# emuell/AFEC

Hardware: AMD Instinct MI355X
Metric: audio frames/sec low-level crawl, 44.1kHz 1024-hop (higher is better)
Workload: dtype f64

## Files before the change

### afec_amd/csrc/afx_frames32.hip

```cpp

#include <hip/hip_runtime.h>

#include "afx_internal.h"
#include "afx_device.h"
#include "afx_fft32.h"

namespace afx {
namespace {

using f32x32::cx;

constexpr int kHalfSlots = 1056;
constexpr int kPlane32Bytes = 2 * kHalfSlots * 8;
constexpr int kWaves32 = 8;

template <int POST_ROWS>
struct Lds32 {
  static constexpr int tw = 0;
  static constexpr int post = tw + 32 * 32 * 16;
  static constexpr int dct = post + POST_ROWS * 32 * 16;
  static constexpr int logc = dct + 14 * 16 * 8;
  static constexpr int xchg = logc + 32 * 8;
  static constexpr int total = xchg + kWaves32 * kPlane32Bytes;
};

__device__ __forceinline__ __amdgpu_buffer_rsrc_t table_rsrc(const void* p, int bytes) {
  return __builtin_amdgcn_make_buffer_rsrc(const_cast<void*>(p), 0, bytes, 0x00020000);
}
typedef unsigned int u32x4_t __attribute__((ext_vector_type(4)));
typedef unsigned int u32x2_t __attribute__((ext_vector_type(2)));
__device__ __forceinline__ double2 table_load2(__amdgpu_buffer_rsrc_t rs, int lane_off, int row_off) {
  return __builtin_bit_cast(double2, __builtin_amdgcn_raw_buffer_load_b128(rs, lane_off, row_off, 0));
}
__device__ __forceinline__ double table_load1(__amdgpu_buffer_rsrc_t rs, int lane_off, int row_off) {
  return __builtin_bit_cast(double, __builtin_amdgcn_raw_buffer_load_b64(rs, lane_off, row_off, 0));
}

template <int IMM, bool NT>
__device__ __forceinline__ void dma_piece(const void* gaddr, unsigned lds_base) {
  if constexpr (NT)
    asm volatile("s_mov_b32 m0, %1\n\ts_nop 0\n\tglobal_load_lds_dwordx4 %0, off offset:%2 nt"
                 :: "v"(gaddr), "s"(lds_base), "n"(IMM) : "memory", "m0");
  else
    asm volatile("s_mov_b32 m0, %1\n\ts_nop 0\n\tglobal_load_lds_dwordx4 %0, off offset:%2"
                 :: "v"(gaddr), "s"(lds_base), "n"(IMM) : "memory", "m0");
}
template <bool NT = true>
__device__ __forceinline__ void dma_hop(const float* g, unsigned lds_plane) {
  dma_piece<0, NT>(g, lds_plane);
  dma_piece<512, NT>(g, lds_plane + 512);
  dma_piece<1024, NT>(g, lds_plane + 1024);
  dma_piece<1536, NT>(g, lds_plane + 1536);
  dma_piece<2048, NT>(g, lds_plane + 2048);
  dma_piece<2560, NT>(g, lds_plane + 2560);
  dma_piece<3072, NT>(g, lds_plane + 3072);
  dma_piece<3584, NT>(g, lds_plane + 3584);
}

__device__ __forceinline__ double mag_sqrt_mel(double xr, double xi, double tiny, double three) {
  const double x = fma(xi, xi, fma(xr, xr, tiny));
  const double r = __builtin_amdgcn_rsq(x);
  const double y = x * r;
  return y * fma(-r, y, three);
}

__device__ __forceinline__ void keep_lane0(double& re, double& im, double own_re, double own_im, unsigned long long lane0_mask) {
  unsigned long long saved;
  asm volatile("s_mov_b64 %2, exec\n\ts_mov_b64 exec, %5\n\tv_mov_b64 %0, %3\n\tv_mov_b64 %1, %4\n\ts_mov_b64 exec, %2"
               : "+v"(re), "+v"(im), "=&s"(saved) : "v"(own_re), "v"(own_im), "s"(lane0_mask));
}

__device__ __forceinline__ double half_sum16(double (&a)[16], int lane) {
#pragma unroll
  for (int i = 0; i < 8; ++i) {
    swap16(a[i], a[i + 8]);
    a[i] += a[i + 8];
  }
  const bool b3 = (lane & 8) != 0, b2 = (lane & 4) != 0, b1 = (lane & 2) != 0;
#pragma unroll
  for (int i = 0; i < 4; ++i) {
    const double keep = b3 ? a[i + 4] : a[i];
    const double send = b3 ? a[i] : a[i + 4];
    a[i] = keep + dpp_mov<kDppRor8>(send);
  }
#pragma unroll
  for (int i = 0; i < 2; ++i) {
    const double keep = b2 ? a[i + 2] : a[i];
    const double send = b2 ? a[i] : a[i + 2];
    a[i] = keep + dpp_mov<kDppHalfMirror>(send);
  }
  const double keep = b1 ? a[1] : a[0];
  const double send = b1 ? a[0] : a[1];
  double z = keep + dpp_mov<kDppXor2>(send);
  z += dpp_mov<kDppXor1>(z);
  return z;
}

__device__ const double kLogConst[32] = {1.0 / 23.0, 1.0 / 21.0, 1.0 / 19.0, 1.0 / 17.0, 1.0 / 15.0, 1.0 / 13.0,
                                         1.0 / 11.0, 1.0 / 9.0,  1.0 / 7.0,  1.0 / 5.0,  1.0 / 3.0,  0.693147180559945309417,
                                         0.70710678118654752440, 2e-42,
                                         1e-20, 32.0, 0.38268343236508984, -0.9238795325112867, 1.0 / 738.0,
                                         (double)(85.0f / 100.0), 43.0, -1.0 / 60.0, (double)1e-12f, 3.0,
                                         1.44269504088896340736, 20.0 / 2.30258509299404568402, 2.2250738585072014e-308, 3.33547137486383e-154 , 511.0, 0.0, 0.0, 0.0};
constexpr int kCEps = 14, kC32 = 15, kCRotRe = 16, kCRotIm = 17, kCRoll = 19, kCSqrtMin = 27, kC511 = 28;

__device__ __forceinline__ double log_lds(double x, const double* c) {
  double m = __builtin_amdgcn_frexp_mant(x);
  int e = __builtin_amdgcn_frexp_exp(x);
  const bool lowhalf = m < c[12];
  m = lowhalf ? m + m : m;
  e = lowhalf ? e - 1 : e;
  const double s = fast_div(m - 1.0, m + 1.0);
  const double z = s * s;
  double p = c[0];
#pragma unroll
  for (int i = 1; i < 11; ++i) p = fma(p, z, c[i]);
  p = fma(p, z, 1.0);
  return fma((double)e, c[11], 2.0 * s * p);
}

__device__ __forceinline__ void finish_mfcc32(double acc, double*& recp, int& left, int stride2, const double* dct,
                                              const double* logc, int lane) {
  const double lg = log_lds(fmax(acc, logc[13]), logc);
  int ln = lane;
  asm volatile("" : "+v"(ln));
  const int n = (ln >> 1) & 15;
  const double2* drow = reinterpret_cast<const double2*>(dct + 16 * (n < kNumCep ? n : 0));
  const int idx = ((ln & 32) + (ln & 1)) << 2;
  const int lo32 = __double2loint(lg), hi32 = __double2hiint(lg);
  double c = 0.0;
#pragma unroll
  for (int m = 0; m < kNumCep; m += 2) {
    const double2 d = drow[m >> 1];
    const double l0 = __hiloint2double(__builtin_amdgcn_ds_bpermute(idx + 8 * m, hi32), __builtin_amdgcn_ds_bpermute(idx + 8 * m, lo32));
    const double l1 = __hiloint2double(__builtin_amdgcn_ds_bpermute(idx + 8 * m + 8, hi32), __builtin_amdgcn_ds_bpermute(idx + 8 * m + 8, lo32));
    c = fma(l0, d.x, c);
    c = fma(l1, d.y, c);
  }
  if (n < kNumCep && left > 0) *recp = c;
  recp += stride2;
  left -= 2;
}

#ifndef AFX_STAMPS
#define AFX_STAMPS 0
#endif
#if AFX_STAMPS
#define AFX_STAMP(i)                                                                           \
  do {                                                                                         \
    unsigned long long t_;                                                                     \
    asm volatile("s_memtime %0\n\ts_waitcnt lgkmcnt(0)" : "=s"(t_));                           \
    stamp_acc[i] += (unsigned)(t_ - stamp_prev);                                               \
    stamp_prev = t_;                                                                           \
  } while (0)
#else
#define AFX_STAMP(i)
#endif


template <int FEAT, bool SCALED>
__global__ __launch_bounds__(kWaves32 * 64) void frames32_kernel(const FrameArgs a) {
  constexpr bool MAGS = (FEAT == 4 || FEAT == 6);
  constexpr bool MAGS_UPPER = (FEAT == 4);
  constexpr int kMelEarly = 4;
  constexpr bool LO_LDS = (FEAT >= 2 && FEAT <= 4) || FEAT == 6;
  constexpr bool kHopNt = !LO_LDS;
  constexpr bool kLoNt = true;
  constexpr bool STATS = (FEAT >= 1 && FEAT <= 3) || FEAT == 5;
  constexpr bool MOMENTS34 = (FEAT != 5);
  constexpr bool PAIRS = STATS;
  constexpr bool STORE = (FEAT == 2 || FEAT == 3);
  constexpr bool UPPER = (FEAT == 3);
  constexpr int MR = (FEAT >= 1) ? 16 : kMel32Rows;
  using Map = Lds32<kMel32Rows>;
  extern __shared__ __align__(16) unsigned char lds_raw[];
  const int lane = threadIdx.x & 63;
  const int wave = __builtin_amdgcn_readfirstlane(threadIdx.x >> 6);
  const int h = lane >> 5, q = lane & 31;

  copy_lds_table(lds_raw + Map::tw, a.tw32, 32 * 32 * 16, threadIdx.x, kWaves32 * 64);
  copy_lds_table(lds_raw + Map::post, a.post32, kMel32Rows * 32 * 16, threadIdx.x, kWaves32 * 64);
  copy_lds_table(lds_raw + Map::dct, a.dct, 14 * 16 * 8, threadIdx.x, kWaves32 * 64);
  copy_lds_table(lds_raw + Map::logc, kLogConst, 32 * 8, threadIdx.x, kWaves32 * 64);
#if AFX_STAMPS
  unsigned stamp_acc[16] = {};
  unsigned long long life_core0, life_real0;
  asm volatile("s_memtime %0\n\ts_memrealtime %1\n\ts_waitcnt lgkmcnt(0)" : "=s"(life_core0), "=s"(life_real0));
  const bool stamping = (wave == 0) && a.stamps != nullptr;
  unsigned long long stamp_prev = 0;
#endif
  __syncthreads();

  const __amdgpu_buffer_rsrc_t win_rs = table_rsrc(a.win32, 32 * 32 * 16);
  const __amdgpu_buffer_rsrc_t mel_rs = table_rsrc(a.melw32, kMel32Pairs * 32 * 8);
  const int q16 = 16 * q, q8 = 8 * q;
  const double2* const tw = reinterpret_cast<const double2*>(lds_raw + Map::tw) + q;
  const double2* const post = reinterpret_cast<const double2*>(lds_raw + Map::post) + q;
  const double* const dct = reinterpret_cast<const double*>(lds_raw + Map::dct);
  const double* const logc = reinterpret_cast<const double*>(lds_raw + Map::logc);
  const int stride2 = 2 * a.lay.stride;
  double* const plane = reinterpret_cast<double*>(lds_raw + Map::xchg + wave * kPlane32Bytes) + kHalfSlots * h;
  double* const pw = plane + q;
  using lds_vdouble = volatile __attribute__((address_space(3))) double;
  lds_vdouble* const pr = (lds_vdouble*)(plane + 33 * q);
  const int partner = (lane & 32) + ((32 - q) & 31);
  const int dh = (lane >> 4) & 1, drow = lane >> 5, dq = 2 * (lane & 15);
  typedef __attribute__((address_space(3))) void lvoid;
  unsigned char* const plane_bytes = lds_raw + Map::xchg + wave * kPlane32Bytes;
  const unsigned plane_lds = __builtin_amdgcn_readfirstlane((unsigned)(size_t)(lvoid*)plane_bytes);
  double k_tiny = 2.2250738585072014e-308, k_three = 3.0;
  unsigned long long k_lane0 = 0x0000000100000001ull;
  asm volatile("" : "+s"(k_tiny), "+s"(k_three), "+s"(k_lane0));
  lds_vdouble* const hop = (lds_vdouble*)(plane_bytes + 256 * h + 8 * q);

  const float* const pcm = reinterpret_cast<const float*>(a.pcm);

  const int n_items = (a.n_chunks + 1) >> 1;
  const int n_static = min((int)(gridDim.x * kWaves32), n_items);
  for (int slot = blockIdx.x * kWaves32 + wave; slot < n_items;) {
    const int ci = 2 * slot + h;
    const bool have = ci < a.n_chunks;
    const Chunk ch = a.chunks[have ? ci : 2 * slot];
    const int nfr = have ? ch.nframes : 0;
    const double sc = ch.scale;
    const int total = max(__builtin_amdgcn_readlane(nfr, 0), __builtin_amdgcn_readlane(nfr, 32));
    const float2* src = reinterpret_cast<const float2*>(pcm + ch.sample_off) + q;
    const int cid = 2 * slot + dh;
    const bool have_d = cid < a.n_chunks;
    const Chunk chd = a.chunks[have_d ? cid : 2 * slot];
    const int last_d = max((have_d ? (int)chd.nframes : 0) - 1, 0);
    const float* const dsrc = pcm + chd.sample_off + 64 * (16 + drow) + 2 * dq;

    double lo[16];
    if constexpr (!LO_LDS) {
      const double* const src8 = reinterpret_cast<const double*>(src);
#pragma unroll
      for (int r = 0; r < 16; ++r) lo[r] = src8[32 * r];
    } else {
      dma_hop<kLoNt>(dsrc - kHop, plane_lds + 8192);
    }
    dma_hop<kHopNt>(dsrc, plane_lds);

    double mel_acc = 0.0;
    double* recp = a.rec + ((int64_t)ch.frame0 + (q & 1)) * a.lay.stride + a.lay.mfcc + ((q >> 1) & 15);
    int left = nfr - (q & 1);

    double2 w[32];
#pragma unroll
    for (int r = 0; r < 32; ++r) w[r] = table_load2(win_rs, q16, 512 * r);

#if AFX_STAMPS
    asm volatile("s_memtime %0\n\ts_waitcnt lgkmcnt(0)" : "=s"(stamp_prev));
#endif
    for (int fi = 0; fi < total; ++fi) {
      cx<double> v[32];
      {
        double nx[16];
        asm volatile("s_waitcnt vmcnt(0)" ::: "memory");
        AFX_STAMP(0);
#pragma unroll
        for (int r = 0; r < 16; ++r) nx[r] = hop[64 * r];
        __builtin_amdgcn_sched_barrier(0);
        if constexpr (LO_LDS) {
          const double* const lo_rows = reinterpret_cast<const double*>(plane_bytes + 8192 + 256 * h) + q;
#pragma unroll
          for (int r = 0; r < 16; ++r) lo[r] = lo_rows[64 * r];
        }
        double hop_sq = 0.0, hop_max = 0.0;
#pragma unroll
        for (int j = 0; j < 8; ++j) {
          auto first = [](double pair) { return __int_as_float(__double2loint(pair)); };
          auto second = [](double pair) { return __int_as_float(__double2hiint(pair)); };
          const double ar = pcm_double<SCALED>(first(lo[j]), sc), ai = pcm_double<SCALED>(second(lo[j]), sc);
          const double br = pcm_double<SCALED>(first(lo[j + 8]), sc), bi = pcm_double<SCALED>(second(lo[j + 8]), sc);
          const double cr = pcm_double<SCALED>(first(nx[j]), sc), ci = pcm_double<SCALED>(second(nx[j]), sc);
          const double dr = pcm_double<SCALED>(first(nx[j + 8]), sc), di = pcm_double<SCALED>(second(nx[j + 8]), sc);
          if constexpr (MAGS) {
            hop_sq = fma(ar, ar, fma(ai, ai, fma(br, br, fma(bi, bi, hop_sq))));
            hop_max = fmax(fmax(hop_max, fmax(fabs(ar), fabs(ai))), fmax(fabs(br), fabs(bi)));
          }
          const double par = ar * w[j].x, pai = ai * w[j].y, pbr = br * w[j + 8].x, pbi = bi * w[j + 8].y;
          const double t0r = fma(cr, w[j + 16].x, par), t0i = fma(ci, w[j + 16].y, pai);
          const double t1r = fma(-cr, w[j + 16].x, par), t1i = fma(-ci, w[j + 16].y, pai);
          const double t2r = fma(dr, w[j + 24].x, pbr), t2i = fma(di, w[j + 24].y, pbi);
          const double t3r = fma(-dr, w[j + 24].x, pbr), t3i = fma(-di, w[j + 24].y, pbi);
          v[j] = {t0r + t2r, t0i + t2i};
          v[j + 16] = {t0r - t2r, t0i - t2i};
          v[j + 8] = {t1r + t3i, t1i - t3r};
          v[j + 24] = {t1r - t3i, t1i + t3r};
        }
        if constexpr (!LO_LDS) {
#pragma unroll
          for (int r = 0; r < 16; ++r) lo[r] = nx[r];
        }
        if constexpr (MAGS) {
          if (a.mask & ((1u << 11) | (1u << 12))) {
            hop_sq += dpp_or_zero<kDppXor1>(hop_sq);      hop_max = fmax(hop_max, dpp_mov<kDppXor1>(hop_max));
            hop_sq += dpp_or_zero<kDppXor2>(hop_sq);      hop_max = fmax(hop_max, dpp_mov<kDppXor2>(hop_max));
            hop_sq += dpp_or_zero<kDppHalfMirror>(hop_sq); hop_max = fmax(hop_max, dpp_mov<kDppHalfMirror>(hop_max));
            hop_sq += dpp_or_zero<kDppMirror>(hop_sq);    hop_max = fmax(hop_max, dpp_mov<kDppMirror>(hop_max));
            const double sq_h = h ? read_lane<32>(hop_sq) + read_lane<48>(hop_sq) : read_lane<0>(hop_sq) + read_lane<16>(hop_sq);
            const double mx_h = h ? fmax(read_lane<32>(hop_max), read_lane<48>(hop_max)) : fmax(read_lane<0>(hop_max), read_lane<16>(hop_max));
            if (q == 0 && fi < nfr) {
              double* const rec = a.rec + ((int64_t)ch.frame0 + fi) * a.lay.stride;
              if ((a.mask & (1u << 11)) && a.lay.amp_peak >= 0) rec[a.lay.amp_peak] = mx_h;
              if ((a.mask & (1u << 12)) && a.lay.amp_rms >= 0) rec[a.lay.amp_rms] = nan_to_zero(sqrt(sq_h / (double)kHop));
            }
          }
        }
      }
      __builtin_amdgcn_sched_barrier(0);
      AFX_STAMP(1);
      f32x32::dft32_rest(v);
      __builtin_amdgcn_sched_barrier(0);
      AFX_STAMP(2);

      double2 t[32];
      auto load_tw = [&](int g) {
#pragma unroll
        for (int j = 2 * g; j < 2 * g + 2; ++j)
#pragma unroll
          for (int i = 0; i < 4; ++i)
            if (j + 8 * i != 0) t[j + 8 * i] = tw[32 * (j + 8 * i)];
      };
      auto bfly_tw = [&](int g) {
#pragma unroll
        for (int j = 2 * g; j < 2 * g + 2; ++j) {
          const cx<double> w1{t[j + 8].x, t[j + 8].y}, w2{t[j + 16].x, t[j + 16].y}, w3{t[j + 24].x, t[j + 24].y};
          if (j == 0) f32x32::radix4_tw3(v[0], v[8], v[16], v[24], w1, w2, w3);
          else f32x32::radix4_tw4(v[j], v[j + 8], v[j + 16], v[j + 24], cx<double>{t[j].x, t[j].y}, w1, w2, w3);
        }
      };
      {
        double re[32], im[32];
#pragma unroll
        for (int k1 = 0; k1 < 32; ++k1) pw[33 * k1] = v[k1].re;
#pragma unroll
        for (int n2 = 0; n2 < 32; ++n2) re[n2] = pr[n2];
#pragma unroll
        for (int k1 = 0; k1 < 32; ++k1) pw[33 * k1] = v[k1].im;
#pragma unroll
        for (int n2 = 0; n2 < 32; ++n2) im[n2] = pr[n2];
        load_tw(0);
        load_tw(1);
#pragma unroll
        for (int n2 = 0; n2 < 32; ++n2) v[n2] = {re[n2], im[n2]};
      }
      asm volatile("s_waitcnt lgkmcnt(0)" ::: "memory");
      AFX_STAMP(3);
      dma_hop<kHopNt>(dsrc + (size_t)min(fi + 1, last_d) * kHop, plane_lds);
      __builtin_amdgcn_sched_barrier(0);

      bfly_tw(0);
      load_tw(2);
      __builtin_amdgcn_sched_barrier(0);
      bfly_tw(1);
      load_tw(3);
      __builtin_amdgcn_sched_barrier(0);
      bfly_tw(2);
      bfly_tw(3);
      __builtin_amdgcn_sched_barrier(0);
      AFX_STAMP(4);
      f32x32::dft32_rest(v);
      __builtin_amdgcn_sched_barrier(0);
      AFX_STAMP(5);

      double mag[MR];
      cx<double> pp[MR];
      double2 pw2[MR];
      double mwt[kMel32Pairs];
      double s1 = 0.0, s2 = 0.0, sj = 0.0, sjj = 0.0, s3 = 0.0, s4 = 0.0, prod_a = 1.0, prod_b = 1.0;
      double jq = 0.0, pa = 0.0;
      double jmir = 0.0;
      double mir[4] = {0.0, 0.0, 0.0, 0.0}, cmid = 0.0;
      double* const park = reinterpret_cast<double*>(plane_bytes + 8192 + 4352 * h);
      auto mag_row = [&]() -> double* {
        int fl = fi, ql = lane;
        asm volatile("" : "+v"(ql), "+s"(fl));
        const int64_t mrow = (fl < nfr) ? (int64_t)ch.frame0 + fl : a.mag_spare_row;
        return a.mag_out + mrow * 1024 + (ql & 31);
      };
      double band26 = 0.0, band27 = 0.0;
      double* rowd = nullptr;
      double* rowm = nullptr;
      auto mag_rows = [&]() {
        rowd = mag_row();
        int ql = lane;
        asm volatile("" : "+v"(ql));
        rowm = rowd + 1024 - 2 * (ql & 31);
      };
      auto store_mag = [&](double* p, double value) { __builtin_nontemporal_store(value > logc[kCSqrtMin] ? value : 0.0, p); };
      if (STATS) {
        int ql = lane;
        asm volatile("" : "+v"(ql));
        jq = (double)((ql & 31) - 1);
        if (PAIRS) jmir = (double)(767 - (ql & 31));
      }
      auto accumulate_at = [&](double value, double j, bool in_range, double* store_at, bool all_in_range) {
        const bool audible = value > logc[kCSqrtMin];
        const bool ok = in_range && audible;
        const double m = ok ? value : 0.0;
        if (STORE && store_at) *store_at = all_in_range ? m : (audible ? value : 0.0);
        const double m2 = m * m;
        const double jm = j * m;
        s1 += m;
        s2 += m2;
        sj += jm;
        sjj = fma(j, jm, sjj);
        if (MOMENTS34) {
          s3 = fma(m2, m, s3);
          s4 = fma(m2, m2, s4);
        }
        prod_b *= ok ? (value + logc[kCEps]) : 1.0;
      };
      auto accumulate = [&](int r, double* store_at) {
        const bool audible = mag[r] > logc[kCSqrtMin];
        const bool ok = ((r == 0) ? (q != 0) : true) && audible;
        const double m = ok ? mag[r] : 0.0;
        if (STORE && store_at) *store_at = (r == 0) ? (audible ? mag[r] : 0.0) : m;
        const double m2 = m * m;
        const double jm = jq * m;
        s1 += m;
        s2 += m2;
        sj += jm;
        sjj = fma(jq, jm, sjj);
        if (MOMENTS34) {
          s3 = fma(m2, m, s3);
          s4 = fma(m2, m2, s4);
        }
        const double f = ok ? (mag[r] + logc[kCEps]) : 1.0;
        if (r < 12) prod_a *= f; else prod_b *= f;
        jq += logc[kC32];
      };
      auto fetch = [&](int r) {
        pp[r] = {__shfl(v[31 - r].re, partner), __shfl(v[31 - r].im, partner)};
        pw2[r] = post[32 * (r % kMel32Rows)];
      };
      auto untangle = [&](int r) {
        cx<double> p = pp[r];
        keep_lane0(p.re, p.im, v[(32 - r) & 31].re, v[(32 - r) & 31].im, k_lane0);
        const cx<double> z = v[r];
        double2 wq = pw2[r];
        if (r >= kMel32Rows) {
          const double cr = logc[kCRotRe], ci = logc[kCRotIm];
          wq = double2{fma(wq.x, cr, -wq.y * ci), fma(wq.x, ci, wq.y * cr)};
        }
        const double er = z.re + p.re, ei = z.im - p.im;
        const double orr = z.im + p.im, oi = p.re - z.re;
        if (MAGS) {
          const double tr = fma(wq.x, orr, -wq.y * oi), ti = fma(wq.x, oi, wq.y * orr);
          const double xr = er + tr, xi = ei + ti, yr = er - tr, yi = ei - ti;
          const double md = mag_sqrt_mel(xr, xi, k_tiny, k_three);
          const double mv = mag_sqrt_mel(yr, yi, k_tiny, k_three);
          if (r < kMel32Rows) park[32 * r + q] = md;
          store_mag(rowd + 32 * r, md);
          if (MAGS_UPPER || r >= 8) {
            if (!(r == 0 && q == 0)) store_mag(rowm - 32 * r, mv);
          }
          if (r <= 8) {
            const double sq = fma(yi, yi, yr * yr);
            if (r < 3) band27 += (r == 0 && q == 0) ? 0.0 : sq;
            else if (r == 3) { band27 += (q <= 23) ? sq : 0.0; band26 += (q <= 23) ? 0.0 : sq; }
            else if (r < 8) band26 += sq;
            else band26 += (q <= 30) ? sq : 0.0;
          }
        } else if (PAIRS && (STORE || r >= 8)) {
          const double tr = fma(wq.x, orr, -wq.y * oi), ti = fma(wq.x, oi, wq.y * orr);
          const double xr = er + tr, xi = ei + ti, yr = er - tr, yi = ei - ti;
          mag[r] = mag_sqrt_mel(xr, xi, k_tiny, k_three);
          if (r < 8) {
            const double sq = fma(yi, yi, yr * yr);
            if (r < 3) band27 += (r == 0 && q == 0) ? 0.0 : sq;
            else if (r == 3) { band27 += (q <= 23) ? sq : 0.0; band26 += (q <= 23) ? 0.0 : sq; }
            else band26 += sq;
            if (UPPER) {
              const double mv = mag_sqrt_mel(yr, yi, k_tiny, k_three);
              double* const dst = mag_row() + (1024 - 32 * r) - 2 * q;
              if (!(r == 0 && q == 0)) *dst = mv > logc[kCSqrtMin] ? mv : 0.0;
            }
          } else {
            const double mv = mag_sqrt_mel(yr, yi, k_tiny, k_three);
            if (r < kMel32Rows) park[32 * (r + 4) + q] = mv;
            else {
              mir[r - kMel32Rows] = mv;
              accumulate_at(mv, jmir, true, STORE ? mag_row() + (1024 - 32 * r) - 2 * q : nullptr, true);
              jmir -= logc[kC32];
            }
          }
        } else {
          const double xr = fma(wq.x, orr, fma(-wq.y, oi, er));
          const double xi = fma(wq.x, oi, fma(wq.y, orr, ei));
          mag[r] = mag_sqrt_mel(xr, xi, k_tiny, k_three);
        }
        if (STATS && r >= kMel32Rows) accumulate(r, STORE ? mag_row() + 32 * r : nullptr);
      };
      if constexpr (MAGS) {
        fetch(0); fetch(1);
        __builtin_amdgcn_sched_barrier(0);
#pragma unroll
        for (int g = 0; g < 8; ++g) {
          if (g < 7) { fetch(2 * g + 2); fetch(2 * g + 3); }
          mag_rows();
          untangle(2 * g);
          untangle(2 * g + 1);
          if (g == kMelEarly) {
#pragma unroll
            for (int i = 0; i < kMel32Pairs; ++i) mwt[i] = table_load1(mel_rs, q8, 256 * i);
          }
          __builtin_amdgcn_sched_barrier(0);
        }
        const double er = v[16].re + v[16].re, orr = v[16].im + v[16].im;
        const double cm = mag_sqrt_mel(er, orr, k_tiny, k_three);
        if (q == 0) store_mag(rowd + 512, cm);
        __builtin_amdgcn_sched_barrier(0);
#pragma unroll
        for (int r = 0; r < kMel32Rows; ++r) mag[r] = park[32 * r + q];
        __builtin_amdgcn_sched_barrier(0);
      } else if constexpr (STATS) {
        fetch(0); fetch(1);
        __builtin_amdgcn_sched_barrier(0);
#pragma unroll
        for (int g = 0; g < 6; ++g) {
          if (g < 5) { fetch(2 * g + 2); fetch(2 * g + 3); }
          untangle(2 * g);
          untangle(2 * g + 1);
          __builtin_amdgcn_sched_barrier(0);
        }
      } else {
#pragma unroll
      for (int r = 0; r < 4; ++r) fetch(r);
      __builtin_amdgcn_sched_barrier(0);
#pragma unroll
      for (int r = 4; r < 8; ++r) fetch(r);
#pragma unroll
      for (int r = 0; r < 4; ++r) untangle(r);
      __builtin_amdgcn_sched_barrier(0);
#pragma unroll
      for (int r = 8; r < 12; ++r) fetch(r);
#pragma unroll
      for (int r = 4; r < 8; ++r) untangle(r);
      __builtin_amdgcn_sched_barrier(0);
      if (FEAT == 0) {
#pragma unroll
        for (int i = 0; i < kMel32Pairs; ++i) mwt[i] = table_load1(mel_rs, q8, 256 * i);
      }
#pragma unroll
      for (int r = 8; r < 12; ++r) untangle(r);
      __builtin_amdgcn_sched_barrier(0);
      }
      if (STATS) {
#pragma unroll
        for (int i = 0; i < kMel32Pairs; ++i) mwt[i] = table_load1(mel_rs, q8, 256 * i);
      }
      AFX_STAMP(6);

      {
        double e[16];
#pragma unroll
        for (int f = 0; f < 16; ++f) e[f] = 0.0;
#pragma unroll
        for (int r = 0; r < kMel32Rows; ++r)
#pragma unroll
          for (int f = 0; f < kNumCep; ++f)
            if (mel32_touches(f, r)) e[f] += mag[r] * mwt[mel32_pair_index(r, f)];
        __builtin_amdgcn_sched_barrier(0);
        AFX_STAMP(7);
        if (STATS) {
          const double tot1 = half_sum16(e, lane);
          if ((lane & 1) == (fi & 1)) mel_acc = tot1;
          {
            double* const row0 = STORE ? mag_row() : nullptr;
#pragma unroll
            for (int r = 0; r < kMel32Rows; ++r) accumulate(r, STORE ? row0 + 32 * r : nullptr);
          }
          {
            double ra[16];
#pragma unroll
            for (int r = 0; r < 16; ++r) ra[r] = (r < 12) ? ((r == 0 && q == 0) ? 0.0 : mag[r]) : 0.0;
            pa = half_sum16(ra, lane);
#pragma unroll
            for (int r = 0; r < 12; ++r) park[32 * r + q] = mag[r];

          }
          __builtin_amdgcn_sched_barrier(0);
#pragma unroll
          for (int r = 12; r < 16; ++r) fetch(r);
          if constexpr (PAIRS) {
            double* const mrow0 = STORE ? mag_row() + 1024 - 2 * q : nullptr;
#pragma unroll
            for (int i = 0; i < 4; ++i) {
              const double mv = park[32 * (12 + i) + q];
              if (STORE && i == 0) band26 += (q <= 30) ? 0.25 * (mv * mv) : 0.0;
              accumulate_at(mv, jmir, (i == 0) ? (q >= 30) : true, STORE ? mrow0 - 32 * (8 + i) : nullptr, i != 0);
              jmir -= logc[kC32];
            }
          }
          __builtin_amdgcn_sched_barrier(0);
#pragma unroll
          for (int r = 12; r < 16; ++r) untangle(r);
          __builtin_amdgcn_sched_barrier(0);
          if constexpr (PAIRS) {
            const double er = v[16].re + v[16].re, orr = v[16].im + v[16].im;
            cmid = (q == 0) ? mag_sqrt_mel(er, orr, k_tiny, k_three) : 0.0;
            accumulate_at(cmid, logc[kC511], q == 0, (STORE && q == 0) ? mag_row() + 512 : nullptr, true);
          }
        }
        if (FEAT == 0 || MAGS) {
#pragma unroll
          for (int r = 0; r < 32; ++r) w[r] = table_load2(win_rs, q16, 512 * r);
          if constexpr (LO_LDS) dma_hop<kLoNt>(dsrc + (size_t)min(fi + 1, last_d) * kHop - kHop, plane_lds + 8192);
        }
        if (FEAT == 0 || MAGS) {
          if (MAGS) {
            e[14] = 4.0 * band26;
            e[15] = 4.0 * band27;
          }
          const double tot = half_sum16(e, lane);
          if ((lane & 1) == (fi & 1)) mel_acc = tot;
          if (MAGS) {
            int ql = lane;
            asm volatile("" : "+v"(ql));
            const int hq = ql & 31;
            double* const rec = a.rec + ((int64_t)ch.frame0 + fi) * a.lay.stride;
            if (fi < nfr && a.lay.bands >= 0 && (hq == 28 || hq == 30)) rec[a.lay.bands + 26 + ((hq - 28) >> 1)] = tot;
          }
        }
        AFX_STAMP(8);
        if (STATS) {
          int ln = lane;
          asm volatile("" : "+v"(ln));
          const int hq = ln & 31;
          double st[16];
          st[0] = s1; st[1] = s2; st[2] = sj; st[3] = sjj; st[4] = s3; st[5] = s4;
          st[6] = log_lds(prod_a, logc) + log_lds(prod_b, logc);
          st[7] = STORE ? 4.0 * band26 : 0.0;
          st[8] = STORE ? 4.0 * band27 : 0.0;
#pragma unroll
          for (int i = 9; i < 16; ++i) st[i] = 0.0;
          const double red = half_sum16(st, ln);
          const int64_t row = (int64_t)ch.frame0 + fi;
          const bool live = fi < nfr;
          double* const tmp = a.stat_tmp + row * kStatTmp;
          if (live && (hq & 1) == 0 && (hq >> 1) < 7) tmp[hq >> 1] = red;
          if (STORE) {
            double* const rec = a.rec + row * a.lay.stride;
            if (live && a.lay.bands >= 0 && (hq == 14 || hq == 16)) rec[a.lay.bands + 26 + ((hq >> 1) - 7)] = red;
          }
          const int base_idx = (ln & 32) << 2;
          const double total = __hiloint2double(__builtin_amdgcn_ds_bpermute(base_idx, __double2hiint(red)),
                                                __builtin_amdgcn_ds_bpermute(base_idx, __double2loint(red)));
          const double pivot = total * logc[kCRoll];
          double rb[16];
          if constexpr (PAIRS) {
#pragma unroll
            for (int r = 0; r < 4; ++r) rb[r] = mag[12 + r];
            rb[4] = cmid;
#pragma unroll
            for (int i = 0; i < 4; ++i) rb[5 + i] = mir[3 - i];
#pragma unroll
            for (int i = 0; i < 4; ++i) rb[9 + i] = (i == 3 && hq < 30) ? 0.0 : park[32 * (15 - i) + hq];
            rb[13] = rb[14] = rb[15] = 0.0;
          }
          double pb = half_sum16(rb, ln);
          pa += dpp_or_zero<kDppRowShr2>(pa);  pb += dpp_or_zero<kDppRowShr2>(pb);
          pa += dpp_or_zero<kDppRowShr4>(pa);  pb += dpp_or_zero<kDppRowShr4>(pb);
          pa += dpp_or_zero<kDppRowShr8>(pa);  pb += dpp_or_zero<kDppRowShr8>(pb);
          pa += dpp_or_zero<kDppRowBcast15, 0xA>(pa);  pb += dpp_or_zero<kDppRowBcast15, 0xA>(pb);
          const int last_idx = base_idx + (22 << 2);
          const double tot_a = __hiloint2double(__builtin_amdgcn_ds_bpermute(last_idx, __double2hiint(pa)),
                                                __builtin_amdgcn_ds_bpermute(last_idx, __double2loint(pa)));
          pb += tot_a;
          const unsigned long long ma = __ballot((hq & 1) == 0 && (hq >> 1) < 12 && pa < pivot);
          const unsigned long long mb = __ballot((hq & 1) == 0 && (hq >> 1) < 13 && pb < pivot);
          const unsigned halfmask_shift = ln & 32;
          const int rstar = __popc((unsigned)(ma >> halfmask_shift)) + __popc((unsigned)(mb >> halfmask_shift));
          const int prev = rstar - 1;
          const int slot = (prev < 12) ? prev : prev - 12;
          const int idx_a = base_idx + ((2 * (slot & 15)) << 2);
          const double base_a = __hiloint2double(__builtin_amdgcn_ds_bpermute(idx_a, __double2hiint(pa)),
                                                 __builtin_amdgcn_ds_bpermute(idx_a, __double2loint(pa)));
          const double base_b = __hiloint2double(__builtin_amdgcn_ds_bpermute(idx_a, __double2hiint(pb)),
                                                 __builtin_amdgcn_ds_bpermute(idx_a, __double2loint(pb)));
          const double before = (rstar == 0) ? 0.0 : ((prev < 12) ? base_a : base_b);
          double xs;
          bool okq;
          int bins_before;
          if constexpr (PAIRS) {
            const bool parked_m = rstar >= 21;
            const int prow = (rstar < 12) ? rstar : (parked_m ? 36 - rstar : 0);
            xs = park[32 * prow + (parked_m ? 31 - hq : hq)];
#pragma unroll
            for (int r = 12; r < 16; ++r) xs = (rstar == r) ? mag[r] : xs;
            xs = (rstar == 16) ? cmid : xs;
            double xm = mir[0];
#pragma unroll
            for (int i = 1; i < 4; ++i) xm = (rstar == 20 - i) ? mir[i] : xm;
            const int ridx = base_idx + ((31 - hq) << 2);
            const double xrev = __hiloint2double(__builtin_amdgcn_ds_bpermute(ridx, __double2hiint(xm)),
                                                 __builtin_amdgcn_ds_bpermute(ridx, __double2loint(xm)));
            xs = (rstar >= 17 && rstar <= 20) ? xrev : xs;
            okq = (rstar == 0) ? (hq != 0) : ((rstar == 16) ? (hq == 0) : ((rstar == 24) ? (hq <= 1) : (rstar < 24)));
            bins_before = (rstar < 16) ? 32 * rstar - (rstar > 0 ? 1 : 0) : ((rstar == 16) ? 511 : 512 + 32 * (rstar - 17));
          }
          xs = okq ? xs : 0.0;
          const double run = halfwave_scan_incl(xs);
          const unsigned long long mrow = __ballot(okq && (before + run) < pivot);
          const int in_row = __popc((unsigned)(mrow >> halfmask_shift));
          const int below = bins_before + in_row;
          int cnt = (pivot > 0.0) ? below + 1 : 0;
          cnt = cnt > kBinCount ? kBinCount : cnt;
          if (live && hq == 0) tmp[7] = (double)cnt;
          __builtin_amdgcn_sched_barrier(0);

#pragma unroll
          for (int r = 0; r < 32; ++r) w[r] = table_load2(win_rs, q16, 512 * r);
          if constexpr (LO_LDS) dma_hop<kLoNt>(dsrc + (size_t)min(fi + 1, last_d) * kHop - kHop, plane_lds + 8192);
        }
        if (fi & 1) finish_mfcc32(mel_acc, recp, left, stride2, dct, logc, lane);
        AFX_STAMP(9);
#if AFX_STAMPS
        stamp_acc[15] += 1;
#endif
      }
    }
    if (total & 1) finish_mfcc32(mel_acc, recp, left, stride2, dct, logc, lane);
    unsigned drawn = 0;
    if (lane == 0) drawn = atomicAdd(a.queue, 1u);
    slot = n_static + (int)((unsigned)__builtin_amdgcn_readfirstlane(drawn) - a.queue_base);
  }
#if AFX_STAMPS
  if (stamping && lane == 0)
    for (int i = 0; i < 16; ++i) atomicAdd(&a.stamps[i], (unsigned long long)stamp_acc[i]);
  if (a.stamps != nullptr && lane == 0) {
    unsigned long long life_core1, life_real1;
    asm volatile("s_memtime %0\n\ts_memrealtime %1\n\ts_waitcnt lgkmcnt(0)" : "=s"(life_core1), "=s"(life_real1));
    unsigned long long* const l = a.stamps + 16 + 4 * ((blockIdx.x & 255) * 8 + wave);
    l[0] = life_core0; l[1] = life_core1; l[2] = life_real0; l[3] = life_real1;
  }
#endif
}

__global__ __launch_bounds__(256) void stats32_finish_kernel(const FrameArgs a, int64_t n_frames) {
  const int64_t f = (int64_t)blockIdx.x * 256 + threadIdx.x;
  if (f >= n_frames) return;
  const double* t = a.stat_tmp + f * kStatTmp;
  const double s1 = t[0], s2 = t[1], sj = t[2], sjj = t[3], s3 = t[4], s4 = t[5], slog = t[6], cnt = t[7];
  double* const rec = a.rec + f * a.lay.stride;
  const double n = (double)kBinCount, inv_n = 1.0 / (double)kBinCount;
  if (a.mask & (1u << 1)) rec[a.lay.srms] = nan_to_zero(sqrt(s2 * inv_n));
  if (a.mask & 0x3Cu) {
    double cen = 0.0, spr = 0.0;
    if (s1 != 0.0) {
      cen = sj / s1;
      spr = (sjj - cen * sj) / s1;
    }
    if (a.lay.centroid >= 0) rec[a.lay.centroid] = cen;
    if (a.lay.spread >= 0) rec[a.lay.spread] = spr;
    if (a.mask & 0x30u) {
      double sk = 0.0, ku = 0.0;
      if (fabs(spr) > (double)1e-12f) {
        const double inv = 1.0 / spr, c2 = cen * cen;
        const double m3 = s3 - 3.0 * cen * s2 + 3.0 * c2 * s1 - n * c2 * cen;
        const double m4 = s4 - 4.0 * cen * s3 + 6.0 * c2 * s2 - 4.0 * c2 * cen * s1 + n * c2 * c2;
        const double i2 = inv * inv;
        sk = m3 * i2 * inv * inv_n;
        ku = m4 * i2 * i2 * inv_n - 3.0;
      }
      if (a.lay.skew >= 0) rec[a.lay.skew] = sk;
      if (a.lay.kurt >= 0) rec[a.lay.kurt] = ku;
    }
  }
  if (a.mask & (1u << 7)) {
    const double gm = fast_exp(slog * inv_n);
    const double am = s1 * inv_n;
    const double fl = (am == 0.0) ? 0.0 : gm / am;
    const double d = lin_to_db(fl) * (-1.0 / 60.0);
    rec[a.lay.flatness] = nan_to_zero(d < 1.0 ? d : 1.0);
  }
  if (a.mask & (1u << 6)) rec[a.lay.rolloff] = cnt * (double)(kSampleRate / (kFft / 2));
}

}

int frames32_waves_per_block() { return kWaves32; }
int frames32_stat_tmp_doubles() { return kStatTmp; }

bool frames_use_halfwave(uint32_t mask, int precision, int pcm_dtype) {
  return (mask & 1u) && !(mask & ~(0x3FFFu | kFramesWholeSpectrum | kFramesStatsLater)) && precision == 0 && (pcm_dtype == kPcmF32 || pcm_dtype == kPcmScaledF32);
}
int frames32_class(uint32_t mask) {
  if (mask == 1u) return 0;
  if (!(mask & ~0xFFu)) return 1;
  if (mask & kFramesStatsLater) return 4;
  return (mask & kFramesWholeSpectrum) ? 3 : 2;
}

template <int FEAT, bool SCALED>
static hipError_t launch_frames32_class(const FrameArgs& a, int grid_blocks, hipStream_t stream) {
  constexpr int lds = Lds32<kMel32Rows>::total;
  auto k = frames32_kernel<FEAT, SCALED>;
  static bool attribute_set[16] = {};
  int dev = 0;
  (void)hipGetDevice(&dev);
  if (dev < 0 || dev >= 16 || !attribute_set[dev]) {
    hipError_t e = hipFuncSetAttribute(reinterpret_cast<const void*>(k), hipFuncAttributeMaxDynamicSharedMemorySize, lds);
    if (e != hipSuccess) return e;
    if (dev >= 0 && dev < 16) attribute_set[dev] = true;
  }
// ... 35 lines not shown
```

### afec_amd/csrc/afx_plan.cpp

```cpp

#include <algorithm>
#include <cmath>
#include <cstring>
#include <new>

#include "afx_host.h"

#ifndef M_PI
#define M_PI 3.14159265358979323846
#endif

namespace afx {
namespace host {

namespace {
thread_local std::string g_last_error;
}

int fail(int status, const std::string& msg) {
  g_last_error = msg;
  return status;
}
int hip_fail(hipError_t e, const char* what) {
  (void)hipGetLastError();
// ... 33 lines not shown
    lin[n] = 700 * (std::exp(mel[n] / 1127) - 1);
    peak[n] = (int)(lin[n] / nyquist * M);
  }
  int cursor = 0;
  for (int n = 0; n < nb; ++n) {
    double* row = tab.data() + (size_t)n * N;
    const double height = 1.0;
    double inc = (n == 0) ? height / peak[n] : height / (peak[n] - peak[n - 1]);
    double val = 0;
    for (int k = 0; k < cursor; ++k) row[k] = 0.0;
    for (; cursor <= peak[n]; ++cursor) {
      row[cursor] = val;
      val += inc;
    }
    inc = height / (peak[n + 1] - peak[n]);
    val = 0;
    for (cursor = peak[n + 1]; cursor > peak[n]; --cursor) {
      row[cursor] = val;
      val += inc;
    }
    for (int k = peak[n + 1] + 1; k < N; ++k) row[k] = 0.0;
  }
  return tab;
}

template <typename T>
struct cpx {
  T re, im;
};

template <typename T>
cpx<T> twiddle(long long e, long long n) {
  e %= n;
  if (e < 0) e += n;
  const long double ang = -2.0L * 3.14159265358979323846264338327950288L * (long double)e / (long double)n;
  return {(T)std::cos(ang), (T)std::sin(ang)};
}

template <typename T>
int upload_tables_typed(afx_plan* p) {
  using C = cpx<T>;
  const int fft = p->desc.fft_size;
  std::vector<C> win(1024), t1(64), t2(1024), post(1024);
  for (int r = 0; r < 16; ++r)
    for (int lane = 0; lane < 64; ++lane) {
      const int n = 64 * r + lane;
      win[n] = {(T)(p->window[2 * n] / (2.0 * fft)), (T)(p->window[2 * n + 1] / (2.0 * fft))};
      post[n] = twiddle<T>(lane + 64 * r, 2048);
    }
  for (int jh = 0; jh < 4; ++jh)
    for (int m2 = 0; m2 < 4; ++m2)
      for (int jl = 0; jl < 4; ++jl) t1[16 * jh + 4 * m2 + jl] = twiddle<T>((long long)m2 * (4 * jh + jl), 64);
  for (int g = 0; g < 16; ++g)
    for (int lane = 0; lane < 64; ++lane) {
      const int j2 = g >> 2, jl = g & 3, jh = lane >> 4, n2 = lane & 15;
      t2[64 * g + lane] = twiddle<T>((long long)n2 * (4 * jh + jl + 16 * j2), 1024);
    }
  auto up = [](void** dst, const void* src, size_t bytes) -> hipError_t {
    hipError_t e = hipMalloc(dst, bytes);
    if (e != hipSuccess) return e;
    return hipMemcpy(*dst, src, bytes, hipMemcpyHostToDevice);
  };
  HIP_TRY(up(&p->dev.win, win.data(), win.size() * sizeof(C)));
  HIP_TRY(up(&p->dev.t1, t1.data(), t1.size() * sizeof(C)));
  HIP_TRY(up(&p->dev.t2, t2.data(), t2.size() * sizeof(C)));
  HIP_TRY(up(&p->dev.post, post.data(), post.size() * sizeof(C)));
  if (sizeof(T) == 8) {
    p->dev.t1_f64 = p->dev.t1; p->dev.t2_f64 = p->dev.t2; p->dev.post_f64 = p->dev.post;
  }
  return AFX_OK;
}

int upload_halfwave_tables(afx_plan* p) {
  using C = cpx<double>;
  const int fft = p->desc.fft_size;
  std::vector<C> win(1024), tw(1024), post(1024);
  for (int r = 0; r < 32; ++r)
    for (int q = 0; q < 32; ++q) {
      const int n = q + 32 * r;
      win[32 * r + q] = {p->window[2 * n] / (4.0 * fft), p->window[2 * n + 1] / (4.0 * fft)};
      tw[32 * r + q] = twiddle<double>((long long)r * q, 1024);
      post[32 * r + q] = twiddle<double>(n, 2048);
    }
  std::vector<double> melw((size_t)afx::kMel32Pairs * 32, 0.0);
  int idx = 0;
  for (int r = 0; r < afx::kMel32Rows; ++r)
    for (int f = 0; f < afx::kNumCep; ++f)
      if (afx::mel32_touches(f, r)) {
        for (int q = 0; q < 32; ++q) melw[(size_t)idx * 32 + q] = p->mel[(size_t)f * afx::kHalf + 32 * r + q];
        ++idx;
      }
  auto up = [](void** dst, const void* src, size_t bytes) -> hipError_t {
    hipError_t e = hipMalloc(dst, bytes);
    if (e != hipSuccess) return e;
    return hipMemcpy(*dst, src, bytes, hipMemcpyHostToDevice);
  };
  HIP_TRY(up(&p->dev.win32, win.data(), win.size() * sizeof(C)));
  HIP_TRY(up(&p->dev.tw32, tw.data(), tw.size() * sizeof(C)));
  HIP_TRY(up(&p->dev.post32, post.data(), post.size() * sizeof(C)));
  HIP_TRY(up(&p->dev.melw32, melw.data(), melw.size() * sizeof(double)));
  return AFX_OK;
}

int upload_rhythm_tables(afx_plan* p) {
  using C = cpx<double>;
  const int n = 512;
  std::vector<double> win((size_t)n);
  const double delta = 1.0 / (double)(n - 1);
  for (int i = 0; i < n; ++i) win[(size_t)i] = 0.5 * (0.5 * (1.0 - std::cos(6.2831853071795864769252867665590 * (double)i * delta)));
  std::vector<C> tw(256), ut(256);
  for (int n2 = 0; n2 < 16; ++n2)
    for (int k1 = 0; k1 < 16; ++k1) tw[(size_t)n2 * 16 + k1] = twiddle<double>((long long)n2 * k1, 256);
  for (int r = 0; r < 16; ++r)
    for (int q = 0; q < 16; ++q) ut[(size_t)r * 16 + q] = twiddle<double>(q + 16 * r, 512);
  std::vector<double> canny(25);
  const double sq = 16.0 * 16.0;
  for (int i = -12; i <= 12; ++i) canny[(size_t)(i + 12)] = (double)i / sq * std::exp(-1.0 * (i * i) / (2.0 * sq));
  std::vector<double> ray((size_t)afx::kRayleighTable);
  const double rayparam = 60. * p->desc.sample_rate / 120. / 128;
  for (int i = 0; i < afx::kRayleighTable; ++i)
    ray[(size_t)i] = ((double)(i + 1.) / (rayparam * rayparam)) * std::exp((-((i + 1.) * (i + 1.)) / (2. * (rayparam * rayparam))));
  auto up = [](double** dst, const void* src, size_t bytes) -> hipError_t {
    hipError_t e = hipMalloc((void**)dst, bytes);
    if (e != hipSuccess) return e;
    return hipMemcpy(*dst, src, bytes, hipMemcpyHostToDevice);
  };
  HIP_TRY(up(&p->dev.rt_window, win.data(), win.size() * sizeof(double)));
  HIP_TRY(up(&p->dev.rt_tw, tw.data(), tw.size() * sizeof(C)));
  HIP_TRY(up(&p->dev.rt_ut, ut.data(), ut.size() * sizeof(C)));
  HIP_TRY(up(&p->dev.rt_canny, canny.data(), canny.size() * sizeof(double)));
  HIP_TRY(up(&p->dev.rt_rayleigh, ray.data(), ray.size() * sizeof(double)));
  return AFX_OK;
}

int upload_tables(afx_plan* p) {
  int st = upload_tables_typed<double>(p);
  if (st != AFX_OK) return st;
  HIP_TRY(hipMalloc(&p->dev.probe, 64));
  if ((st = upload_halfwave_tables(p)) != AFX_OK) return st;
  if ((st = upload_rhythm_tables(p)) != AFX_OK) return st;
  std::vector<double> melw((size_t)afx::kMelPairs * 64, 0.0);
  int idx = 0;
  for (int r = 0; r < afx::kMelRows; ++r)
    for (int f = 0; f < afx::kNumCep; ++f)
      if (afx::mel_touches(f, r)) {
        for (int lane = 0; lane < 64; ++lane)
          melw[(size_t)idx * 64 + lane] = p->mel[(size_t)f * afx::kHalf + 64 * r + lane];
        ++idx;
      }
  HIP_TRY(hipMalloc(&p->dev.melw, melw.size() * sizeof(double)));
  HIP_TRY(hipMemcpy(p->dev.melw, melw.data(), melw.size() * sizeof(double), hipMemcpyHostToDevice));
  std::vector<double> dct(14 * 16, 0.0);
  for (int n = 0; n < 14; ++n)
    for (int m = 1; m <= 14; ++m) dct[16 * n + (m - 1)] = std::cos(M_PI * (n / (double)14) * (m - 0.5));
  HIP_TRY(hipMalloc((void**)&p->dev.dct, dct.size() * sizeof(double)));
  HIP_TRY(hipMemcpy(p->dev.dct, dct.data(), dct.size() * sizeof(double), hipMemcpyHostToDevice));
  return AFX_OK;
}

void free_tables(afx_plan* p) {
  if (p->dev.t1_f64 != p->dev.t1) { hipFree(p->dev.t1_f64); hipFree(p->dev.t2_f64); hipFree(p->dev.post_f64); }
  hipFree(p->dev.win); hipFree(p->dev.t1); hipFree(p->dev.t2); hipFree(p->dev.post);
  hipFree(p->dev.melw); hipFree(p->dev.dct);
  hipFree(p->dev.win32); hipFree(p->dev.tw32); hipFree(p->dev.post32); hipFree(p->dev.melw32);
  hipFree(p->dev.rt_window); hipFree(p->dev.rt_tw); hipFree(p->dev.rt_ut); hipFree(p->dev.rt_canny); hipFree(p->dev.rt_rayleigh);
  hipFree(p->dev.rs_filter);
  hipFree(p->dev.probe);
  p->dev = DeviceTables{};
}

}

// ... 235 lines not shown
```

Baseline: 512.9 million.

## Widen LDS and table loads to 128-bit and restructure PCM/MFCC exchange paths

After: 533.8 million, median of 6. +4.1%, better.

```diff
diff --git a/afec_amd/csrc/afx_frames32.hip b/afec_amd/csrc/afx_frames32.hip
--- a/afec_amd/csrc/afx_frames32.hip
+++ b/afec_amd/csrc/afx_frames32.hip
@@ -10,9 +10,15 @@
 
 using f32x32::cx;
 
-constexpr int kHalfSlots = 1056;
+constexpr int kRowSlots = 34;
+constexpr int kHalfSlots = kRowSlots * 32;
 constexpr int kPlane32Bytes = 2 * kHalfSlots * 8;
+constexpr int kMel32Loads = (kMel32Pairs + 1) / 2;
 constexpr int kWaves32 = 8;
+
+using lds_vdouble = volatile __attribute__((address_space(3))) double;
+typedef double f64x2_t __attribute__((ext_vector_type(2)));
+using lds_vdouble2 = volatile __attribute__((address_space(3))) f64x2_t;
 
 template <int POST_ROWS>
 struct Lds32 {
@@ -31,9 +37,6 @@
 typedef unsigned int u32x2_t __attribute__((ext_vector_type(2)));
 __device__ __forceinline__ double2 table_load2(__amdgpu_buffer_rsrc_t rs, int lane_off, int row_off) {
   return __builtin_bit_cast(double2, __builtin_amdgcn_raw_buffer_load_b128(rs, lane_off, row_off, 0));
-}
-__device__ __forceinline__ double table_load1(__amdgpu_buffer_rsrc_t rs, int lane_off, int row_off) {
-  return __builtin_bit_cast(double, __builtin_amdgcn_raw_buffer_load_b64(rs, lane_off, row_off, 0));
 }
 
 template <int IMM, bool NT>
@@ -119,23 +122,37 @@
   return fma((double)e, c[11], 2.0 * s * p);
 }
 
+template <bool VIA_LDS>
 __device__ __forceinline__ void finish_mfcc32(double acc, double*& recp, int& left, int stride2, const double* dct,
-                                              const double* logc, int lane) {
+                                              const double* logc, int lane, unsigned char* bcast) {
   const double lg = log_lds(fmax(acc, logc[13]), logc);
   int ln = lane;
   asm volatile("" : "+v"(ln));
   const int n = (ln >> 1) & 15;
   const double2* drow = reinterpret_cast<const double2*>(dct + 16 * (n < kNumCep ? n : 0));
-  const int idx = ((ln & 32) + (ln & 1)) << 2;
-  const int lo32 = __double2loint(lg), hi32 = __double2hiint(lg);
   double c = 0.0;
-#pragma unroll
-  for (int m = 0; m < kNumCep; m += 2) {
-    const double2 d = drow[m >> 1];
-    const double l0 = __hiloint2double(__builtin_amdgcn_ds_bpermute(idx + 8 * m, hi32), __builtin_amdgcn_ds_bpermute(idx + 8 * m, lo32));
-    const double l1 = __hiloint2double(__builtin_amdgcn_ds_bpermute(idx + 8 * m + 8, hi32), __builtin_amdgcn_ds_bpermute(idx + 8 * m + 8, lo32));
-    c = fma(l0, d.x, c);
-    c = fma(l1, d.y, c);
+  if constexpr (VIA_LDS) {
+    unsigned char* const row = bcast + 384 * (ln >> 5) + 192 * (ln & 1);
+    *(lds_vdouble*)(row + 8 * n) = lg;
+    lds_vdouble2* const pairs = (lds_vdouble2*)row;
+#pragma unroll
+    for (int m = 0; m < kNumCep; m += 2) {
+      const double2 d = drow[m >> 1];
+      const f64x2_t l = pairs[m >> 1];
+      c = fma(l.x, d.x, c);
+      c = fma(l.y, d.y, c);
+    }
+  } else {
+    const int idx = ((ln & 32) + (ln & 1)) << 2;
+    const int lo32 = __double2loint(lg), hi32 = __double2hiint(lg);
+#pragma unroll
+    for (int m = 0; m < kNumCep; m += 2) {
+      const double2 d = drow[m >> 1];
+      const double l0 = __hiloint2double(__builtin_amdgcn_ds_bpermute(idx + 8 * m, hi32), __builtin_amdgcn_ds_bpermute(idx + 8 * m, lo32));
+      const double l1 = __hiloint2double(__builtin_amdgcn_ds_bpermute(idx + 8 * m + 8, hi32), __builtin_amdgcn_ds_bpermute(idx + 8 * m + 8, lo32));
+      c = fma(l0, d.x, c);
+      c = fma(l1, d.y, c);
+    }
   }
   if (n < kNumCep && left > 0) *recp = c;
   recp += stride2;
@@ -192,8 +209,8 @@
   __syncthreads();
 
   const __amdgpu_buffer_rsrc_t win_rs = table_rsrc(a.win32, 32 * 32 * 16);
-  const __amdgpu_buffer_rsrc_t mel_rs = table_rsrc(a.melw32, kMel32Pairs * 32 * 8);
-  const int q16 = 16 * q, q8 = 8 * q;
+  const __amdgpu_buffer_rsrc_t mel_rs = table_rsrc(a.melw32, kMel32Loads * 32 * 16);
+  const int q16 = 16 * q;
   const double2* const tw = reinterpret_cast<const double2*>(lds_raw + Map::tw) + q;
   const double2* const post = reinterpret_cast<const double2*>(lds_raw + Map::post) + q;
   const double* const dct = reinterpret_cast<const double*>(lds_raw + Map::dct);
@@ -201,10 +218,9 @@
   const int stride2 = 2 * a.lay.stride;
   double* const plane = reinterpret_cast<double*>(lds_raw + Map::xchg + wave * kPlane32Bytes) + kHalfSlots * h;
   double* const pw = plane + q;
-  using lds_vdouble = volatile __attribute__((address_space(3))) double;
-  lds_vdouble* const pr = (lds_vdouble*)(plane + 33 * q);
+  lds_vdouble2* const pr = (lds_vdouble2*)(plane + kRowSlots * q);
   const int partner = (lane & 32) + ((32 - q) & 31);
-  const int dh = (lane >> 4) & 1, drow = lane >> 5, dq = 2 * (lane & 15);
+  const int dh = (lane >> 4) & 1;
   typedef __attribute__((address_space(3))) void lvoid;
   unsigned char* const plane_bytes = lds_raw + Map::xchg + wave * kPlane32Bytes;
   const unsigned plane_lds = __builtin_amdgcn_readfirstlane((unsigned)(size_t)(lvoid*)plane_bytes);
@@ -224,12 +240,14 @@
     const int nfr = have ? ch.nframes : 0;
     const double sc = ch.scale;
     const int total = max(__builtin_amdgcn_readlane(nfr, 0), __builtin_amdgcn_readlane(nfr, 32));
-    const float2* src = reinterpret_cast<const float2*>(pcm + ch.sample_off) + q;
+    int lc = lane;
+    asm volatile("" : "+v"(lc));
+    const float2* src = reinterpret_cast<const float2*>(pcm + ch.sample_off) + (lc & 31);
     const int cid = 2 * slot + dh;
     const bool have_d = cid < a.n_chunks;
     const Chunk chd = a.chunks[have_d ? cid : 2 * slot];
     const int last_d = max((have_d ? (int)chd.nframes : 0) - 1, 0);
-    const float* const dsrc = pcm + chd.sample_off + 64 * (16 + drow) + 2 * dq;
+    const float* const dsrc = pcm + chd.sample_off + 64 * (16 + (lc >> 5)) + 4 * (lc & 15);
 
     double lo[16];
     if constexpr (!LO_LDS) {
@@ -242,8 +260,8 @@
     dma_hop<kHopNt>(dsrc, plane_lds);
 
     double mel_acc = 0.0;
-    double* recp = a.rec + ((int64_t)ch.frame0 + (q & 1)) * a.lay.stride + a.lay.mfcc + ((q >> 1) & 15);
-    int left = nfr - (q & 1);
+    double* recp = a.rec + ((int64_t)ch.frame0 + (lc & 1)) * a.lay.stride + a.lay.mfcc + ((lc >> 1) & 15);
+    int left = nfr - (lc & 1);
 
     double2 w[32];
 #pragma unroll
@@ -254,14 +272,41 @@
 #endif
     for (int fi = 0; fi < total; ++fi) {
       cx<double> v[32];
-      {
+      auto first = [](double pair) { return __int_as_float(__double2loint(pair)); };
+      auto second = [](double pair) { return __int_as_float(__double2hiint(pair)); };
+      if constexpr (!LO_LDS) {
+        asm volatile("s_waitcnt vmcnt(0)" ::: "memory");
+        AFX_STAMP(0);
+        double par[8], pai[8], pbr[8], pbi[8];
+#pragma unroll
+        for (int j = 0; j < 8; ++j) {
+          const double ar = pcm_double<SCALED>(first(lo[j]), sc), ai = pcm_double<SCALED>(second(lo[j]), sc);
+          const double br = pcm_double<SCALED>(first(lo[j + 8]), sc), bi = pcm_double<SCALED>(second(lo[j + 8]), sc);
+          par[j] = ar * w[j].x, pai[j] = ai * w[j].y, pbr[j] = br * w[j + 8].x, pbi[j] = bi * w[j + 8].y;
+        }
+#pragma unroll
+        for (int r = 0; r < 16; ++r) lo[r] = hop[64 * r];
+#pragma unroll
+        for (int j = 0; j < 8; ++j) {
+          const double cr = pcm_double<SCALED>(first(lo[j]), sc), ci = pcm_double<SCALED>(second(lo[j]), sc);
+          const double dr = pcm_double<SCALED>(first(lo[j + 8]), sc), di = pcm_double<SCALED>(second(lo[j + 8]), sc);
+          const double t0r = fma(cr, w[j + 16].x, par[j]), t0i = fma(ci, w[j + 16].y, pai[j]);
+          const double t1r = fma(-cr, w[j + 16].x, par[j]), t1i = fma(-ci, w[j + 16].y, pai[j]);
+          const double t2r = fma(dr, w[j + 24].x, pbr[j]), t2i = fma(di, w[j + 24].y, pbi[j]);
+          const double t3r = fma(-dr, w[j + 24].x, pbr[j]), t3i = fma(-di, w[j + 24].y, pbi[j]);
+          v[j] = {t0r + t2r, t0i + t2i};
+          v[j + 16] = {t0r - t2r, t0i - t2i};
+          v[j + 8] = {t1r + t3i, t1i - t3r};
+          v[j + 24] = {t1r - t3i, t1i + t3r};
+        }
+      } else {
         double nx[16];
         asm volatile("s_waitcnt vmcnt(0)" ::: "memory");
         AFX_STAMP(0);
 #pragma unroll
         for (int r = 0; r < 16; ++r) nx[r] = hop[64 * r];
         __builtin_amdgcn_sched_barrier(0);
-        if constexpr (LO_LDS) {
+        {
           const double* const lo_rows = reinterpret_cast<const double*>(plane_bytes + 8192 + 256 * h) + q;
 #pragma unroll
           for (int r = 0; r < 16; ++r) lo[r] = lo_rows[64 * r];
@@ -269,8 +314,6 @@
         double hop_sq = 0.0, hop_max = 0.0;
 #pragma unroll
         for (int j = 0; j < 8; ++j) {
-          auto first = [](double pair) { return __int_as_float(__double2loint(pair)); };
-          auto second = [](double pair) { return __int_as_float(__double2hiint(pair)); };
           const double ar = pcm_double<SCALED>(first(lo[j]), sc), ai = pcm_double<SCALED>(second(lo[j]), sc);
           const double br = pcm_double<SCALED>(first(lo[j + 8]), sc), bi = pcm_double<SCALED>(second(lo[j + 8]), sc);
           const double cr = pcm_double<SCALED>(first(nx[j]), sc), ci = pcm_double<SCALED>(second(nx[j]), sc);
@@ -288,10 +331,6 @@
           v[j + 16] = {t0r - t2r, t0i - t2i};
           v[j + 8] = {t1r + t3i, t1i - t3r};
           v[j + 24] = {t1r - t3i, t1i + t3r};
-        }
-        if constexpr (!LO_LDS) {
-#pragma unroll
-          for (int r = 0; r < 16; ++r) lo[r] = nx[r];
         }
         if constexpr (MAGS) {
           if (a.mask & ((1u << 11) | (1u << 12))) {
@@ -334,13 +373,21 @@
       {
         double re[32], im[32];
 #pragma unroll
-        for (int k1 = 0; k1 < 32; ++k1) pw[33 * k1] = v[k1].re;
-#pragma unroll
-        for (int n2 = 0; n2 < 32; ++n2) re[n2] = pr[n2];
-#pragma unroll
-        for (int k1 = 0; k1 < 32; ++k1) pw[33 * k1] = v[k1].im;
-#pragma unroll
-        for (int n2 = 0; n2 < 32; ++n2) im[n2] = pr[n2];
+        for (int k1 = 0; k1 < 32; ++k1) pw[kRowSlots * k1] = v[k1].re;
+#pragma unroll
+        for (int m = 0; m < 16; ++m) {
+          const f64x2_t two = pr[m];
+          re[2 * m] = two.x;
+          re[2 * m + 1] = two.y;
+        }
+#pragma unroll
+        for (int k1 = 0; k1 < 32; ++k1) pw[kRowSlots * k1] = v[k1].im;
+#pragma unroll
+        for (int m = 0; m < 16; ++m) {
+          const f64x2_t two = pr[m];
+          im[2 * m] = two.x;
+          im[2 * m + 1] = two.y;
+        }
         load_tw(0);
         load_tw(1);
 #pragma unroll
@@ -368,7 +415,15 @@
       double mag[MR];
       cx<double> pp[MR];
       double2 pw2[MR];
-      double mwt[kMel32Pairs];
+      double mwt[2 * kMel32Loads];
+      auto load_mel = [&]() {
+#pragma unroll
+        for (int i = 0; i < kMel32Loads; ++i) {
+          const double2 two = table_load2(mel_rs, q16, 512 * i);
+          mwt[2 * i] = two.x;
+          mwt[2 * i + 1] = two.y;
+        }
+      };
       double s1 = 0.0, s2 = 0.0, sj = 0.0, sjj = 0.0, s3 = 0.0, s4 = 0.0, prod_a = 1.0, prod_b = 1.0;
       double jq = 0.0, pa = 0.0;
       double jmir = 0.0;
@@ -504,8 +559,7 @@
           untangle(2 * g);
           untangle(2 * g + 1);
           if (g == kMelEarly) {
-#pragma unroll
-            for (int i = 0; i < kMel32Pairs; ++i) mwt[i] = table_load1(mel_rs, q8, 256 * i);
+            load_mel();
           }
           __builtin_amdgcn_sched_barrier(0);
         }
@@ -541,16 +595,14 @@
       for (int r = 4; r < 8; ++r) untangle(r);
       __builtin_amdgcn_sched_barrier(0);
       if (FEAT == 0) {
-#pragma unroll
-        for (int i = 0; i < kMel32Pairs; ++i) mwt[i] = table_load1(mel_rs, q8, 256 * i);
+        load_mel();
       }
 #pragma unroll
       for (int r = 8; r < 12; ++r) untangle(r);
       __builtin_amdgcn_sched_barrier(0);
       }
       if (STATS) {
-#pragma unroll
-        for (int i = 0; i < kMel32Pairs; ++i) mwt[i] = table_load1(mel_rs, q8, 256 * i);
+        load_mel();
       }
       AFX_STAMP(6);
 
@@ -716,14 +768,14 @@
           for (int r = 0; r < 32; ++r) w[r] = table_load2(win_rs, q16, 512 * r);
           if constexpr (LO_LDS) dma_hop<kLoNt>(dsrc + (size_t)min(fi + 1, last_d) * kHop - kHop, plane_lds + 8192);
         }
-        if (fi & 1) finish_mfcc32(mel_acc, recp, left, stride2, dct, logc, lane);
+        if (fi & 1) finish_mfcc32<FEAT == 0>(mel_acc, recp, left, stride2, dct, logc, lane, plane_bytes + 8192);
         AFX_STAMP(9);
 #if AFX_STAMPS
         stamp_acc[15] += 1;
 #endif
       }
     }
-    if (total & 1) finish_mfcc32(mel_acc, recp, left, stride2, dct, logc, lane);
+    if (total & 1) finish_mfcc32<FEAT == 0>(mel_acc, recp, left, stride2, dct, logc, lane, plane_bytes + 8192);
     unsigned drawn = 0;
     if (lane == 0) drawn = atomicAdd(a.queue, 1u);
     slot = n_static + (int)((unsigned)__builtin_amdgcn_readfirstlane(drawn) - a.queue_base);
diff --git a/afec_amd/csrc/afx_plan.cpp b/afec_amd/csrc/afx_plan.cpp
--- a/afec_amd/csrc/afx_plan.cpp
+++ b/afec_amd/csrc/afx_plan.cpp
@@ -139,12 +139,12 @@
       tw[32 * r + q] = twiddle<double>((long long)r * q, 1024);
       post[32 * r + q] = twiddle<double>(n, 2048);
     }
-  std::vector<double> melw((size_t)afx::kMel32Pairs * 32, 0.0);
+  std::vector<double> melw((size_t)((afx::kMel32Pairs + 1) / 2) * 64, 0.0);
   int idx = 0;
   for (int r = 0; r < afx::kMel32Rows; ++r)
     for (int f = 0; f < afx::kNumCep; ++f)
       if (afx::mel32_touches(f, r)) {
-        for (int q = 0; q < 32; ++q) melw[(size_t)idx * 32 + q] = p->mel[(size_t)f * afx::kHalf + 32 * r + q];
+        for (int q = 0; q < 32; ++q) melw[(size_t)(idx >> 1) * 64 + 2 * q + (idx & 1)] = p->mel[(size_t)f * afx::kHalf + 32 * r + q];
         ++idx;
       }
   auto up = [](void** dst, const void* src, size_t bytes) -> hipError_t {
```
